# Francis-Fan-create/SCaSML_GP

Hardware: AMD Instinct MI355X
Metric: Euler-Maruyama path-steps/sec + L2 rel-error, Grad_Dependent_Nonlinear d=100 n=3 (higher is better)
Workload: dtype f32

## Files before the change

scasml_gp_amd/csrc/gp_eval_compat_mfma.hip:

```cpp
#include <stdlib.h>
#include <type_traits>

#include "gp_common.hpp"
#include "gp_mfma16.hpp"

namespace scasml {

constexpr int kHutch = 5;

typedef _Float16 h16x2 __attribute__((ext_vector_type(2)));
typedef float f32x2 __attribute__((ext_vector_type(2)));

struct CompatIdxF {
    int32_t i[kHutch];
};

struct GpCompatArgs {
    const float *points;
    const float *model;
    int32_t idx[kHutch];
    float4 *out4;
    float *lap;
    int64_t n_inf;
    int32_t n_pad, kp, d, first_bdy_tile;
    float a, sigma, mu;
    int32_t eq_id;
    int32_t round_out;
    const uint8_t *site_kinds;
    int64_t rows_per_site;
    const int32_t *site_order;
    int32_t n_listed;
    int32_t tail_packed;
};

template <bool R16>
struct Pair {
    using T = std::conditional_t<R16, h16x2, f32x2>;
    T v;
    __device__ __forceinline__ Pair(float a, float b) {
        if constexpr (R16) v = __builtin_convertvector((f32x2){a, b}, h16x2);
        else v = (f32x2){a, b};
    }
    __device__ __forceinline__ float lo() const { return (float)v.x; }
    __device__ __forceinline__ float hi() const { return (float)v.y; }
};

__device__ __forceinline__ float pin(float x) {
    asm("" : "+v"(x));
    return x;
}

static inline bool compat_tail_packed(int d, int kp) {
    const int r = d + 1 - (kp - 16);
    return 2 * (r > 0 ? r : 0) + 4 <= 16;
}

template <int KS, int PLANES, bool PACK>
__device__ __forceinline__ void compat_mfma_lam(const float4 *lds_a, const s16x8 (&xb)[PLANES][KS], f32x16 &acc, int lane, float acc0) {
#pragma unroll
    for (int r = 0; r < 16; ++r) acc[r] = acc0;
    constexpr int NA = PLANES == 2 ? 1 : 2;
    Frag a[NA];
    if constexpr (NA == 2) a[0].f = lds_a[lane];
#pragma unroll
    for (int s = 0; s < KS; ++s) {
        const int cur = NA == 2 ? (s & 1) : 0, nxt = cur ^ 1;
        if constexpr (NA == 2) {
            if (s + 1 < KS) a[nxt].f = lds_a[(s + 1) * 64 + lane];
        } else {
            a[0].f = lds_a[s * 64 + lane];
        }
        Frag b0;
        b0.v = xb[0][s];
        if constexpr (PLANES == 2) {
            if (!(PACK && s == KS - 1)) {
                Frag b1;
                b1.v = xb[1][s];
                acc = __builtin_amdgcn_mfma_f32_32x32x16_f16(a[cur].h, b1.h, acc, 0, 0, 0);
            }
        }
        acc = __builtin_amdgcn_mfma_f32_32x32x16_f16(a[cur].h, b0.h, acc, 0, 0, 0);
        __builtin_amdgcn_sched_barrier(0);
    }
}

struct CompatPoint {
    float sx, tx, ax0, sx2, wxa, wxb;
};
struct CompatConsts {
    float a, ad, c4, c10;
};

template <int GEOM, int FORM, bool BDY, bool R16>
__device__ __forceinline__ void compat_epilogue(const float *rows_lds, const f32x16 &lam, const f32x16 &G, int half, const CompatPoint &p,
                                                const CompatConsts &c, float &au, float &at, float &ad, float &al) {
    const float4 *cb = reinterpret_cast<const float4 *>(__builtin_assume_aligned(rows_lds + 4 * 8 * half, 16));
    constexpr int NQ = (BDY || GEOM == 1) ? 1 : 2;
    float4 q[1][NQ];
    auto fetch = [&](int r, float4 (&dst)[NQ]) {
        const int row = (r & 3) + 8 * (r >> 2);
#pragma unroll
        for (int i = 0; i < NQ; ++i) dst[i] = cb[row * 2 + i];
    };
#pragma unroll
    for (int r = 0; r < 16; ++r) {
        const int cur = 0;
        fetch(r, q[0]);
        __builtin_amdgcn_sched_barrier(0);
        const float kap = pin(__builtin_amdgcn_exp2f(lam[r]));
        if constexpr (GEOM == 0) {
            const float vsy = q[cur][0].x, vty = q[cur][0].y, c0 = q[cur][0].z;
            if constexpr (BDY && FORM == 1) {
                const Pair<R16> k0(kap, 0.0f);
                au = fmaf(c0, k0.lo(), au);
            } else {
                const float pp = p.tx - vty, ss = p.sx - vsy;
                const float e1 = pin(pp * kap), e2 = pin(ss * kap);
                if constexpr (BDY) {
                    const Pair<R16> k01(kap, e1), k2(e2, 0.0f);
                    au = fmaf(c0, k01.lo(), au);
                    if constexpr (FORM == 0) at = fmaf(-c0, k01.hi(), at);
                    if constexpr (FORM != 1) ad = fmaf(-c0, k2.lo(), ad);
                } else {
                    const float cL = q[cur][0].w, ct = q[cur][1].x, cS = q[cur][1].y;
                    if constexpr (FORM == 1) {
                        const Pair<R16> k01(kap, e1), k2(e2, 0.0f);
                        au = fmaf(cS, k2.lo(), fmaf(ct, k01.hi(), fmaf(c0, k01.lo(), au)));
                    } else {
                        const float e4 = pin(pp * e2);
                        const float e5 = pin(fmaf(-ss, e2, c.ad * kap));
                        if constexpr (FORM == 2) {
                            const Pair<R16> k01(kap, e1), k24(e2, e4), k5(e5, 0.0f);
                            au = fmaf(cS, k24.lo(), fmaf(ct, k01.hi(), fmaf(c0, k01.lo(), au)));
                            ad = fmaf(cS, k5.lo(), fmaf(-ct, k24.hi(), fmaf(-c0, k24.lo(), ad)));
                        } else {
                            const float e3 = fmaf(-pp, e1, c.a * kap);
                            const float g0 = G[r];
                            const float e6 = fmaf(g0, g0 - c.c4, -c.c10) * kap;
                            const Pair<R16> k01(kap, e1), k23(e2, e3), k45(e4, e5), k6(e6, 0.0f);
                            au = fmaf(cS, k23.lo(), fmaf(ct, k01.hi(), fmaf(c0, k01.lo(), au)));
                            at = fmaf(-cS, k45.lo(), fmaf(ct, k23.hi(), fmaf(-c0, k01.hi(), at)));
                            ad = fmaf(cS, k45.hi(), fmaf(-ct, k45.lo(), fmaf(-c0, k23.lo(), ad)));
                            al = fmaf(cL, k6.lo(), al);
                        }
                    }
                }
            }
        } else if constexpr (GEOM == 1) {
            const float vsy1 = q[cur][0].x, vay0 = q[cur][0].y, vwy1 = q[cur][0].z, cL = q[cur][0].w;
            const float g1 = G[r];
            const float f1 = pin(g1 * kap);
            if constexpr (FORM == 1) {
                const Pair<R16> k1(f1, 0.0f);
                au = fmaf(cL, k1.lo(), au);
            } else {
                const float m = fmaf(-(p.sx - vsy1), g1, p.wxb - vwy1);
                const float f3 = pin(m * kap);
                if constexpr (FORM == 2) {
                    const Pair<R16> k13(f1, f3);
                    au = fmaf(cL, k13.lo(), au);
                    ad = fmaf(cL, k13.hi(), ad);
                } else {
                    const float f2 = (p.tx - vay0) * f1;
                    const Pair<R16> k12(f1, f2), k3(f3, 0.0f);
                    au = fmaf(cL, k12.lo(), au);
                    at = fmaf(-cL, k12.hi(), at);
                    ad = fmaf(cL, k3.lo(), ad);
                }
            }
        } else {
            const float vsy = q[cur][0].x, vty = q[cur][0].y, vwy2 = q[cur][0].z, c0 = q[cur][0].w;
            const float g2 = G[r];
            const float h1 = g2 * kap;
            if constexpr (BDY) {
                const Pair<R16> k1(h1, 0.0f);
                al = fmaf(c0, k1.lo(), al);
            } else {
                const float ct = q[cur][1].x, cS = q[cur][1].y;
                const float h2 = (p.ax0 - vty) * h1;
                const float m = fmaf(-(p.sx2 - vsy), g2, p.wxa - vwy2);
                const float h3 = m * kap;
                const Pair<R16> k12(h1, h2), k3(h3, 0.0f);
                al = fmaf(-cS, k3.lo(), fmaf(ct, k12.hi(), fmaf(c0, k12.lo(), al)));
            }
        }
    }
}

template <int GEOM, int FORM, bool BDY>
__device__ __forceinline__ void compat_epilogue_fact(const float *rows_lds, const f32x16 &lam, const f32x16 &G, int half, const CompatPoint &p,
                                                     const CompatConsts &c, float &au, float &at, float &ad, float &al) {
    const float4 *cb = reinterpret_cast<const float4 *>(__builtin_assume_aligned(rows_lds + 4 * 8 * half, 16));
    constexpr int Q0 = GEOM == 2 ? 1 : 0;
    constexpr int NQ = (GEOM == 0 && !BDY) ? 2 : 1;
    float4 q[2][NQ];
    auto fetch = [&](int r, float4 (&dst)[NQ]) {
        const int row = (r & 3) + 8 * (r >> 2);
#pragma unroll
        for (int i = 0; i < NQ; ++i) dst[i] = cb[row * 2 + Q0 + i];
    };
    fetch(0, q[0]);
#pragma unroll
    for (int r = 0; r < 16; ++r) {
        const int cur = r & 1, nxt = cur ^ 1;
        if (r + 1 < 16) fetch(r + 1, q[nxt]);
        #ifndef SCASML_FACT_NOSCHED
        __builtin_amdgcn_sched_barrier(0);
#endif
        const float kap = __builtin_amdgcn_exp2f(lam[r]);
        if constexpr (GEOM == 0) {
            const float vsy = q[cur][0].x, vty = q[cur][0].y, c0 = q[cur][0].z;
            if constexpr (BDY) {
                const float F = c0 * kap;
                au += F;
                if constexpr (FORM == 0) at = fmaf(-(p.tx - vty), F, at);
                if constexpr (FORM != 1) ad = fmaf(-(p.sx - vsy), F, ad);
            } else {
                const float cL = q[cur][0].w, ct = q[cur][1].x, cS = q[cur][1].y;
                const float pp = p.tx - vty, ss = p.sx - vsy;
                const float E = fmaf(ct, pp, fmaf(cS, ss, c0));
                au = fmaf(kap, E, au);
                if constexpr (FORM != 1) ad = fmaf(kap, fmaf(-ss, E, q[cur][1].w), ad);
                if constexpr (FORM == 0) {
                    at = fmaf(kap, fmaf(-pp, E, q[cur][1].z), at);
                    const float g0 = G[r];
                    al = fmaf(cL * kap, fmaf(g0, g0 - c.c4, -c.c10), al);
                }
            }
        } else if constexpr (GEOM == 1) {
            const float vsy1 = q[cur][0].x, vay0 = q[cur][0].y, vwy1 = q[cur][0].z, cL = q[cur][0].w;
            const float v = cL * kap;
            if constexpr (FORM == 1) {
                au = fmaf(v, G[r], au);
            } else {
                const float w = v * G[r];
                au += w;
                ad = fmaf(-(p.sx - vsy1), w, fmaf(v, p.wxb - vwy1, ad));
                if constexpr (FORM == 0) at = fmaf(-(p.tx - vay0), w, at);
            }
        } else {
            const float ct = q[cur][0].x, cS = q[cur][0].y, e0 = q[cur][0].z, cSw = q[cur][0].w;
            if constexpr (BDY) {
                al = fmaf(kap * G[r], e0, al);
            } else {
                const float E2 = fmaf(ct, p.ax0, fmaf(cS, p.sx2, e0));
                const float t = fmaf(cS, p.wxa, -cSw);
                al = fmaf(kap, fmaf(G[r], E2, -t), al);
            }
        }
    }
}

constexpr int kStageTail = 256 + 256;

template <int KS, bool R16, int PLANES, bool PACK>
__device__ __forceinline__ void compat_mfma_sweep(const GpCompatArgs g) {
    static_assert(PLANES == 2 || !R16, "the as-coded form keeps both point planes");
#ifndef SCASML_COMPAT_NSLOT
#define SCASML_COMPAT_NSLOT 3
#endif
    constexpr int WPB = 4, NSLOT = SCASML_COMPAT_NSLOT, AHEAD = 2;
    constexpr int STAGE = KS * 256 + kStageTail;
    constexpr int NCHUNK = STAGE / 256;
    constexpr int CLO = NCHUNK / WPB, CREM = NCHUNK % WPB;
    extern __shared__ __attribute__((aligned(16))) float lds[];
    const int lane = threadIdx.x & 63, wv = threadIdx.x >> 6;
    const int col = lane & 31, half = lane >> 5;
    const int64_t blk = blockIdx.x;
    int64_t p0 = (blk * WPB + wv) * 32;
    const int n_tiles = g.n_pad / 32;
    const int nb0 = g.first_bdy_tile < n_tiles ? g.first_bdy_tile : n_tiles;

    int form_listed = -1;
    if (g.site_order) {
        const int64_t wps = g.rows_per_site >> 5;
        bool all_u = true, all_ud = true;
        for (int w = 0; w < WPB; ++w) {
            const int64_t vs = (blk * WPB + w) / wps;
            if (vs >= g.n_listed) continue;
            const int k = g.site_kinds ? g.site_kinds[g.site_order[vs]] : 0;
            if (!(k == 1 || k == 3)) all_u = false;
            if (!(k == 1 || k == 3 || k == 4)) all_ud = false;
        }
        form_listed = all_u ? 1 : (all_ud ? 2 : 0);
        const int64_t vw = blk * WPB + wv, vs = vw / wps;
        p0 = vs < g.n_listed ? (int64_t)g.site_order[vs] * g.rows_per_site + (vw - vs * wps) * 32 : g.n_inf;
    }

    p0 = ((int64_t)__builtin_amdgcn_readfirstlane((int32_t)(p0 >> 32)) << 32) | (uint32_t)__builtin_amdgcn_readfirstlane((int32_t)p0);

    if (!g.site_order && g.site_kinds && g.rows_per_site >= 32) {
        const int64_t b0 = blk * WPB * 32;
        if (b0 < g.n_inf) {
            const int64_t b1 = (b0 + WPB * 32 < g.n_inf ? b0 + WPB * 32 : g.n_inf) - 1;
            bool unowned = true;
            for (int64_t s = b0 / g.rows_per_site; s <= b1 / g.rows_per_site; ++s)
                if (g.site_kinds[s] != 2) unowned = false;
            if (unowned) return;
        }
    }
    int form = 0;
    if (g.site_order) {
        form = form_listed;
    } else if (g.site_kinds && g.rows_per_site >= 32) {
        const int64_t b0 = blk * WPB * 32;
        const int64_t b1 = (b0 + WPB * 32 < g.n_inf ? b0 + WPB * 32 : g.n_inf) - 1;
        if (b0 < g.n_inf) {
            bool all_u = true, all_ud = true;
            for (int64_t s = b0 / g.rows_per_site; s <= b1 / g.rows_per_site; ++s) {
                const int k = g.site_kinds[s];
                if (k == 2) continue;
                if (!(k == 1 || k == 3)) all_u = false;
                if (!(k == 1 || k == 3 || k == 4)) all_ud = false;
            }
            form = all_u ? 1 : (all_ud ? 2 : 0);
        }
    }
    form = __builtin_amdgcn_readfirstlane(form);
    const int GD = form == 0 ? 3 : 2, GB = form == 0 ? 2 : 1;
    const int n_stages = nb0 * GD + (n_tiles - nb0) * GB;

    const int wvs = __builtin_amdgcn_readfirstlane(wv);
    const bool extra = wvs < CREM;
    const uint32_t lds_base = __builtin_amdgcn_readfirstlane((uint32_t)(uintptr_t)lds);
    auto stage_src = [&](int s) -> const float * {
        int tile, geom;
        if (s < nb0 * GD) {
            tile = s / GD;
            geom = s - tile * GD;
        } else {
            const int t = s - nb0 * GD;
            tile = nb0 + t / GB;
            geom = form == 0 ? 2 * (t - (t / GB) * GB) : 0;
        }
        return g.model + ((int64_t)tile * 3 + geom) * STAGE;
    };
    auto stage = [&](int s) {
        const uint32_t dst = lds_base + (uint32_t)((s % NSLOT) * STAGE) * 4u;
        const float *src = stage_src(s);
        auto chunk = [&](int c) { glds16_asm(src + c * 256, (uint32_t)lane * 16u, dst + (uint32_t)c * 1024u); };
#pragma unroll
        for (int i = 0; i < CLO; ++i) chunk(wvs + i * WPB);
        if (CREM && extra) chunk(wvs + CLO * WPB);
    };
    auto rendezvous = [&](bool newest_may_fly) {
        if (newest_may_fly) {
            if (CREM && extra) {
                asm volatile("s_waitcnt vmcnt(%0)" ::"n"(CLO + 1) : "memory");
            } else {
                asm volatile("s_waitcnt vmcnt(%0)" ::"n"(CLO) : "memory");
            }
        } else {
            asm volatile("s_waitcnt vmcnt(0)" ::: "memory");
        }
        __builtin_amdgcn_s_barrier();
        asm volatile("" ::: "memory");
    };
    stage(0);
    if (n_stages > 1) stage(1);

    const float qs = 0.5f * 1.44269504088896341f / g.a, k1 = -qs;
    const float hh = (float)g.d / (float)kHutch;
    const float ha2 = hh * g.a * g.a;
    s16x8 xb[PLANES][KS];
    float acc0 = 0.0f;
    CompatPoint pt;
    Frag qa[1], qb[1];
    {
        int64_t row = p0 + col;
        if (row >= g.n_inf) row = g.n_inf - 1;
        const float *prow = g.points + row * g.kp;
        const float4 *src = reinterpret_cast<const float4 *>(prow + half * (8 * (KS - 1)));
        const float4 *src_tail = reinterpret_cast<const float4 *>(prow + 16 * (KS - 1) + (PACK ? 0 : 8 * half));
        float pn = 0.0f, ps = 0.0f;
        const float ptime = prow[g.d], px0 = prow[0];
        const float fold = 2.0f * g.a * g.a * qs;
        auto lo = [](float v) { return v - (float)(_Float16)v; };
        auto make_planes = [&](const float (&t)[8], Frag &fh, Frag &fl) {
#pragma unroll
            for (int c = 0; c < 4; ++c) {
                fh.u[c] = pack_h2(t[2 * c], t[2 * c + 1]);
                fl.u[c] = pack_h2(lo(t[2 * c]), lo(t[2 * c + 1]));
            }
        };
        float tlast[8];
#pragma unroll
        for (int s = 0; s < KS; ++s) {
            const bool last = s == KS - 1;
            const float4 q0 = last ? src_tail[0] : src[2 * s], q1 = last ? src_tail[1] : src[2 * s + 1];
            const float e[8] = {q0.x, q0.y, q0.z, q0.w, q1.x, q1.y, q1.z, q1.w};
            float t[8];
#pragma unroll
            for (int c2 = 0; c2 < 8; ++c2) {
                const float w = (PACK && last && half) ? 0.0f : e[c2];
                pn = fmaf(w, w, pn);
                ps += w;
                t[c2] = fold * e[c2];
            }
            if (last) {
#pragma unroll
                for (int c2 = 0; c2 < 8; ++c2) tlast[c2] = t[c2];
            } else {
                Frag fh, fl;
                make_planes(t, fh, fl);
                xb[0][s] = fh.v;
                if constexpr (PLANES == 2) xb[1][s] = fl.v;
            }
        }
        pn += __shfl_xor(pn, 32);
        ps += __shfl_xor(ps, 32);
        const float x2 = k1 * g.a * g.a * pn;
        if constexpr (PLANES == 1) {
            const bool packed = g.tail_packed != 0;
            tlast[5] = half ? (packed ? 0.0f : 1.0f) : tlast[5];
            tlast[6] = half ? (packed ? x2 : 1.0f) : (packed ? 1.0f : tlast[6]);
            tlast[7] = half ? (packed ? 0.0f : x2) : (packed ? 1.0f : tlast[7]);
            Frag fh, fl;
            make_planes(tlast, fh, fl);
            xb[0][KS - 1] = fh.v;
            acc0 = lo(x2);
        } else if constexpr (PACK) {
            Frag f;
#pragma unroll
            for (int c = 0; c < 3; ++c) {
                const uint32_t h2 = pack_h2(tlast[2 * c], tlast[2 * c + 1]);
                const uint32_t l2 = pack_h2(lo(tlast[2 * c]), lo(tlast[2 * c + 1]));
                f.u[c] = half ? l2 : h2;
            }
            f.u[3] = half ? pack_h2(x2, lo(x2)) : pack_h2(1.0f, 1.0f);
            xb[0][KS - 1] = f.v;
        } else {
            tlast[5] = half ? 1.0f : tlast[5];
            tlast[6] = half ? 1.0f : tlast[6];
            tlast[7] = half ? x2 : tlast[7];
            Frag fh, fl;
            make_planes(tlast, fh, fl);
            xb[0][KS - 1] = fh.v;
            xb[1][KS - 1] = fl.v;
        }
        pt.sx = g.a * (ps - ptime);
        pt.tx = g.a * ptime;
        pt.ax0 = g.a * px0;
        pt.sx2 = pt.sx - pt.ax0 + pt.tx;
        float ua[kHutch], ub[kHutch], sa = 0.0f, sb = 0.0f, na = 0.0f, nb = 0.0f;
#pragma unroll
        for (int j = 0; j < kHutch; ++j) {
            const float va = prow[g.idx[j] + 1], vb = prow[g.idx[j]];
            sa += va;
            sb += vb;
            na = fmaf(va, va, na);
            nb = fmaf(vb, vb, nb);
            ua[j] = -2.0f * ha2 * va;
            ub[j] = -2.0f * ha2 * vb;
        }
        pt.wxa = 2.0f * ha2 * sa;
        pt.wxb = 2.0f * ha2 * sb;
        auto qfrag = [&](const float (&u)[kHutch], float px, Frag &f) {
            auto hi = [](float v) { return (float)(_Float16)v; };
            if (half == 0) {
                f.u[0] = pack_h2(u[0], u[1]);
                f.u[1] = pack_h2(u[2], u[3]);
                f.u[2] = pack_h2(u[4], px);
                f.u[3] = pack_h2(px - hi(px), 1.0f);
            } else {
                f.u[0] = pack_h2(u[0] - hi(u[0]), u[1] - hi(u[1]));
                f.u[1] = pack_h2(u[2] - hi(u[2]), u[3] - hi(u[3]));
                f.u[2] = pack_h2(u[4] - hi(u[4]), 1.0f);
                f.u[3] = 0u;
            }
        };
        const float c5ah = (float)kHutch * g.a * hh;
        qfrag(ua, fmaf(ha2, na, -c5ah), qa[0]);
        qfrag(ub, fmaf(ha2, nb, -c5ah), qb[0]);
    }
    CompatConsts cc;
    cc.a = g.a;
    cc.ad = g.a * (float)g.d;
    cc.c4 = 4.0f * g.a * hh;
    cc.c10 = 10.0f * g.a * g.a * hh * hh;
    float au = 0.0f, at = 0.0f, ad = 0.0f, al = 0.0f;
    f32x16 acc, accG;
    uint32_t region;
    asm volatile("s_mov_b32 %0, -1" : "=s"(region));

    int s_now = 0;
    auto step = [&](auto geom_c, auto form_c, auto bdy_c) {
        constexpr int GEOM = decltype(geom_c)::value, FORM = decltype(form_c)::value;
        constexpr bool BDY = decltype(bdy_c)::value;
        constexpr bool NEEDG = GEOM != 0 || (FORM == 0 && !BDY);
        const int slot = s_now % NSLOT;
        if (s_now + AHEAD < n_stages) stage(s_now + AHEAD);
        const float *base = lds + slot * STAGE;
        if (region & 1) {
            compat_mfma_lam<KS, PLANES, PACK>(reinterpret_cast<const float4 *>(base), xb, acc, lane, acc0);
            if constexpr (NEEDG) {
                Frag aq;
                aq.f = reinterpret_cast<const float4 *>(base + KS * 256)[lane];
#pragma unroll
                for (int r = 0; r < 16; ++r) accG[r] = 0.0f;
                accG = __builtin_amdgcn_mfma_f32_32x32x16_f16(aq.h, GEOM == 1 ? qb[0].h : qa[0].h, accG, 0, 0, 0);
            }
        }
        if (region & 2) {
            if constexpr (R16) compat_epilogue<GEOM, FORM, BDY, true>(base + (KS + 1) * 256, acc, accG, half, pt, cc, au, at, ad, al);
            else compat_epilogue_fact<GEOM, FORM, BDY>(base + (KS + 1) * 256, acc, accG, half, pt, cc, au, at, ad, al);
        }
        rendezvous(s_now + AHEAD < n_stages);
        ++s_now;
    };
    using I0 = std::integral_constant<int, 0>;
    using I1 = std::integral_constant<int, 1>;
    using I2 = std::integral_constant<int, 2>;
    auto sweep = [&](auto form_c) {
        constexpr int FORM = decltype(form_c)::value;
        for (int jt = 0; jt < nb0; ++jt) {
            step(I0{}, form_c, std::false_type{});
            step(I1{}, form_c, std::false_type{});
            if constexpr (FORM == 0) step(I2{}, form_c, std::false_type{});
        }
        for (int jt = nb0; jt < n_tiles; ++jt) {
            step(I0{}, form_c, std::true_type{});
            if constexpr (FORM == 0) step(I2{}, form_c, std::true_type{});
        }
    };
    rendezvous(n_stages > 1);
    if (form == 2) sweep(I2{});
    else if (form == 1) sweep(I1{});
    else sweep(I0{});

    float u = au + __shfl_xor(au, 32);
    const float dt = at + __shfl_xor(at, 32);
    const float dv = ad + __shfl_xor(ad, 32);
    const float lp = al + __shfl_xor(al, 32);
    int col_out = col;
    if constexpr (R16) asm volatile("" : "+v"(col_out));
    const int64_t row = p0 + col_out;
    if (half == 0 && row < g.n_inf) {
        if (g.round_out) u = (float)(_Float16)u;
        float eps = dt + g.mu * dv + 0.5f * g.sigma * g.sigma * lp + eq_f<float>(g.eq_id, u, g.sigma * dv, g.sigma, (float)g.d);
        if (g.round_out) eps = (float)(_Float16)eps;
        g.out4[row] = make_float4(u, dv, eps, dt);
        if (g.lap) g.lap[row] = lp;
    }
}

template <int KS, int BPC, bool R16, int PLANES>
__global__ __launch_bounds__(256, BPC) void gp_eval_compat_mfma_kernel(const GpCompatArgs g) {
    compat_mfma_sweep<KS, R16, PLANES, false>(g);
}

template <int KS, int BPC, bool R16, int PLANES>
__global__ __launch_bounds__(256, BPC) void gp_eval_compat_mfma_tail_kernel(const GpCompatArgs g) {
    compat_mfma_sweep<KS, R16, PLANES, true>(g);
}

__global__ void gp_compat_pack_mfma_kernel(int d, float a, const float *x_dom, int n_dom, const float *x_bdy, int n_bdy, const double *rv,
                                           CompatIdxF ix, float *model, int n_pad, int kp, int packed) {
    const int j = blockIdx.x * blockDim.x + threadIdx.x;
    if (j >= n_pad) return;
    const int N = n_dom + n_bdy, D = d + 1, KS = kp / 16;
    const float *src = j < n_dom ? x_dom + (int64_t)j * D : (j < N ? x_bdy + (int64_t)(j - n_dom) * D : nullptr);
    auto y = [&](int k) { return src ? src[k] : 0.0f; };
    const float qs = 0.5f * 1.44269504088896341f / a, k1 = -qs;
    const float hh = (float)d / (float)kHutch, ha2 = hh * a * a;
    float ny = 0.0f, sy = 0.0f;
    for (int k = 0; k < D; ++k) ny = fmaf(y(k), y(k), ny);
    for (int k = 0; k < d; ++k) sy += y(k);
    const float ay = k1 * a * a * ny;
    const _Float16 ayh = (_Float16)ay;
    const float ayl = ay - (float)ayh;
    float c0 = 0.0f, cL = 0.0f, ct = 0.0f, cS = 0.0f;
    if (j < n_dom) {
        c0 = (float)rv[j];
        cL = (float)rv[N + j];
        ct = (float)rv[N + n_dom + j];
        cS = (float)rv[N + 2 * n_dom + j];
    } else if (j < N) {
        c0 = (float)rv[j];
    }
    const int tile = j / 32, i = j % 32;
    const int stage_floats = KS * 256 + kStageTail;
    for (int g = 0; g < 3; ++g) {
        float *blk = model + ((int64_t)tile * 3 + g) * stage_floats;
        uint16_t *planes = reinterpret_cast<uint16_t *>(blk);
        auto yg = [&](int k) { return g == 0 ? y(k) : (g == 1 ? y((k + 1) % D) : y((k + D - 1) % D)); };
        for (int s = 0; s < KS; ++s) {
            for (int c = 0; c < 16; ++c) {
                const int k = s < KS - 1 ? (c >> 3) * 8 * (KS - 1) + 8 * s + (c & 7)
                                         : 16 * s + (packed && c >= 8 ? c - 8 : c);
                float v = k <= d ? yg(k) : 0.0f;
                if (s == KS - 1) {
                    if (packed) v = (c & 7) < 6 ? v : (c == 6 ? (float)ayh : (c == 7 ? ayl : 1.0f));
                    else v = c < 13 ? v : (c == 13 ? (float)ayh : (c == 14 ? ayl : 1.0f));
                }
                planes[(((int64_t)s * 64 + (c >> 3) * 32 + i) * 8) + (c & 7)] = __builtin_bit_cast(unsigned short, (_Float16)v);
            }
        }
        float yq[kHutch], nq = 0.0f, sq = 0.0f;
        for (int q = 0; q < kHutch; ++q) {
            yq[q] = y(ix.i[q] + (g == 2 ? 0 : 1));
            nq = fmaf(yq[q], yq[q], nq);
            sq += yq[q];
        }
        const float py = ha2 * nq;
        const _Float16 pyh = (_Float16)py;
        uint16_t *qf = reinterpret_cast<uint16_t *>(blk + KS * 256);
        auto put = [&](int h, int e, float v) { qf[(h * 32 + i) * 8 + e] = __builtin_bit_cast(unsigned short, (_Float16)v); };
        for (int q = 0; q < kHutch; ++q) {
            put(0, q, yq[q]);
            put(1, q, yq[q]);
        }
        put(0, 5, 1.0f);
        put(0, 6, 1.0f);
        put(0, 7, (float)pyh);
        put(1, 5, py - (float)pyh);
        put(1, 6, 0.0f);
        put(1, 7, 0.0f);
        float *rc = blk + (KS + 1) * 256 + i * 8;
        for (int q = 0; q < 8; ++q) rc[q] = 0.0f;
        if (g == 0) {
            rc[0] = a * sy;
            rc[1] = a * y(d);
            rc[2] = c0;
            rc[3] = cL;
            rc[4] = ct;
            rc[5] = cS;
            rc[6] = a * ct;
            rc[7] = a * (float)d * cS;
        } else if (g == 1) {
            rc[0] = a * (sy - y(0) + y(d));
            rc[1] = a * y(0);
            rc[2] = 2.0f * ha2 * sq;
            rc[3] = cL;
        } else {
            rc[0] = a * sy;
            rc[1] = a * y(d);
            rc[2] = 2.0f * ha2 * sq;
            rc[3] = c0;
            rc[4] = ct;
            rc[5] = cS;
            rc[6] = fmaf(-cS, rc[0], fmaf(-ct, rc[1], c0));
            rc[7] = cS * rc[2];
        }
    }
}

template <int KS, bool R16, int PLANES, bool PACK>
static int launch_compat(const GpCompatArgs &g, hipStream_t s) {
    constexpr int REGS = 4 * PLANES * KS + (R16 ? 72 : 90);
    constexpr size_t lds_bytes = SCASML_COMPAT_NSLOT * (size_t)(KS * 256 + kStageTail) * sizeof(float);
    constexpr int BPC_REGS = REGS <= 128 ? 4 : (REGS <= 164 ? 3 : 2), BPC_LDS = (int)(160 * 1024 / lds_bytes);
    constexpr int BPC = BPC_REGS < BPC_LDS ? BPC_REGS : BPC_LDS;
    const int64_t waves = g.site_order ? (int64_t)g.n_listed * (g.rows_per_site >> 5) : (g.n_inf + 31) / 32;
    const int64_t blocks = (waves + 3) / 4;
    if (blocks == 0) return 0;
    if (blocks > 0x7FFFFFFF) return fail(SCASML_ERR_UNSUPPORTED, "gp_eval_compat_sites: too many points");
    static_assert(lds_bytes * BPC <= 160 * 1024, "LDS slots exceed 160 KiB");
    void (*kern)(const GpCompatArgs) = gp_eval_compat_mfma_kernel<KS, BPC, R16, PLANES>;
    if constexpr (PACK) kern = gp_eval_compat_mfma_tail_kernel<KS, BPC, R16, PLANES>;
    static_assert(PLANES == 2 || !PACK, "one plane: one kernel for both column maps");
    if (lds_bytes > 64 * 1024) {
        if (hipFuncSetAttribute(reinterpret_cast<const void *>(kern), hipFuncAttributeMaxDynamicSharedMemorySize, (int)lds_bytes) != hipSuccess)
            return fail(SCASML_ERR_HIP, "gp_eval_compat_sites: cannot reserve %zu bytes of LDS", lds_bytes);
    }
    hipLaunchKernelGGL(kern, dim3((unsigned)blocks), dim3(256), lds_bytes, s, g);
    return check_launch("gp_eval_compat_sites launch");
}

template <bool R16, int PLANES>
static int launch_compat_ks(const GpCompatArgs &g, hipStream_t s) {
    const bool packed = PLANES == 2 && g.tail_packed;
    switch (g.kp / 16) {
#define SCASML_CASE(K) \
    case K:                                                                                \
        if constexpr (PLANES == 2) {                                                       \
            if (packed) return launch_compat<K, R16, PLANES, true>(g, s);                   \
        }                                                                                  \
        return launch_compat<K, R16, PLANES, false>(g, s);
        SCASML_CASE(1) SCASML_CASE(2) SCASML_CASE(3) SCASML_CASE(4) SCASML_CASE(5) SCASML_CASE(6) SCASML_CASE(7) SCASML_CASE(8)
        SCASML_CASE(9) SCASML_CASE(10) SCASML_CASE(11) SCASML_CASE(12) SCASML_CASE(13) SCASML_CASE(14) SCASML_CASE(15) SCASML_CASE(16)
#undef SCASML_CASE
    }
    return fail(SCASML_ERR_UNSUPPORTED, "gp_eval_compat_sites: kp=%d", g.kp);
}

static int check_idx5(const int32_t *idx_h, int d, int32_t (&out)[kHutch], const char *who) {
    if (!idx_h) return fail(SCASML_ERR_ARG, "%s: idx is null", who);
    for (int j = 0; j < kHutch; ++j) {
        if (idx_h[j] < 0 || idx_h[j] >= d) return fail(SCASML_ERR_ARG, "%s: idx[%d] = %d outside [0, d)", who, j, idx_h[j]);
        for (int q = 0; q < j; ++q)
            if (idx_h[q] == idx_h[j]) return fail(SCASML_ERR_ARG, "%s: idx has a repeated entry %d", who, idx_h[j]);
        out[j] = idx_h[j];
    }
    return 0;
}

}

using namespace scasml;

extern "C" int64_t scasml_gp_compat_model_floats(int32_t d, int32_t n_pad) {
    const int64_t kp = scasml_point_stride(d);
    return (int64_t)(n_pad / SCASML_GP_TILE) * 3 * ((kp / 16) * 256 + kStageTail);
}

extern "C" int scasml_gp_compat_pack_mfma(int32_t d, float a, const float *x_dom, int32_t n_dom, const float *x_bdy, int32_t n_bdy,
                                          const double *rv, const int32_t *idx_h, float *model_out, void *stream) {
    if (!x_dom || !rv || !model_out || (n_bdy > 0 && !x_bdy)) return fail(SCASML_ERR_ARG, "gp_compat_pack_mfma: null argument");
    if (d < kHutch || d > SCASML_MAX_DIM || n_dom < 1 || n_bdy < 0) return fail(SCASML_ERR_ARG, "gp_compat_pack_mfma: bad sizes (d >= %d needed)", kHutch);
    CompatIdxF ix;
    if (int rc = check_idx5(idx_h, d, ix.i, "gp_compat_pack_mfma")) return rc;
    const int n_pad = (n_dom + n_bdy + 31) / 32 * 32;
    const int kp = scasml_point_stride(d);
    hipLaunchKernelGGL(gp_compat_pack_mfma_kernel, dim3((n_pad + 63) / 64), dim3(64), 0, (hipStream_t)stream, d, a, x_dom, n_dom, x_bdy, n_bdy,
                       rv, ix, model_out, n_pad, kp, compat_tail_packed(d, kp) ? 1 : 0);
    return check_launch("gp_compat_pack_mfma launch");
}

static int eval_compat_sites(int32_t d, float a, float sigma_eq, float mu_eq, int32_t eq_id, const float *model, int32_t n_dom,
                             int32_t n_bdy, const int32_t *idx_h, int32_t round16, float x_bound, const float *points, int64_t n_inf,
                             int64_t rows_per_site, const uint8_t *site_kinds, const int32_t *site_order, int32_t n_listed, float *out4, float *lap,
                             void *stream);

extern "C" int scasml_gp_eval_compat_sites(int32_t d, float a, float sigma_eq, float mu_eq, int32_t eq_id, const float *model, int32_t n_dom,
                                           int32_t n_bdy, const int32_t *idx_h, int32_t round16, float x_bound, const float *points, int64_t n_inf,
                                           int64_t rows_per_site, const uint8_t *site_kinds, float *out4, float *lap, void *stream) {
    return eval_compat_sites(d, a, sigma_eq, mu_eq, eq_id, model, n_dom, n_bdy, idx_h, round16, x_bound, points, n_inf, rows_per_site, site_kinds, nullptr,
                             0, out4, lap, stream);
}

extern "C" int scasml_gp_eval_compat_site_list(int32_t d, float a, float sigma_eq, float mu_eq, int32_t eq_id, const float *model, int32_t n_dom,
                                               int32_t n_bdy, const int32_t *idx_h, int32_t round16, float x_bound, const float *points, int64_t n_inf,
                                               int64_t rows_per_site, const uint8_t *site_kinds, const int32_t *site_order, int32_t n_listed,
                                               float *out4, float *lap, void *stream) {
    if (!site_order || n_listed < 0) return fail(SCASML_ERR_ARG, "gp_eval_compat_site_list: null or negative site list");
    if (rows_per_site < 32 || (rows_per_site & 31)) return fail(SCASML_ERR_ARG, "gp_eval_compat_site_list: rows_per_site must be a positive multiple of 32");
    if (n_inf % rows_per_site) return fail(SCASML_ERR_ARG, "gp_eval_compat_site_list: n_inf must be a whole number of sites");
    if (n_listed > n_inf / rows_per_site) return fail(SCASML_ERR_ARG, "gp_eval_compat_site_list: %d listed sites, the buffer holds %lld", n_listed, (long long)(n_inf / rows_per_site));
    if (n_listed == 0) return 0;
    return eval_compat_sites(d, a, sigma_eq, mu_eq, eq_id, model, n_dom, n_bdy, idx_h, round16, x_bound, points, n_inf, rows_per_site, site_kinds, site_order,
                             n_listed, out4, lap, stream);
}

static int eval_compat_sites(int32_t d, float a, float sigma_eq, float mu_eq, int32_t eq_id, const float *model, int32_t n_dom,
                             int32_t n_bdy, const int32_t *idx_h, int32_t round16, float x_bound, const float *points, int64_t n_inf,
                             int64_t rows_per_site, const uint8_t *site_kinds, const int32_t *site_order, int32_t n_listed, float *out4, float *lap,
                             void *stream) {
    if (n_inf == 0) return 0;
    if (!model || !points || !out4 || n_inf < 0) return fail(SCASML_ERR_ARG, "gp_eval_compat_sites: bad argument");
    if (d < kHutch || d > SCASML_MAX_DIM || n_dom < 1 || n_bdy < 0) return fail(SCASML_ERR_ARG, "gp_eval_compat_sites: bad sizes");
    if (site_kinds && rows_per_site < 1) return fail(SCASML_ERR_ARG, "gp_eval_compat_sites: rows_per_site must be positive");
    if (!eq_known(eq_id)) return fail(SCASML_ERR_UNSUPPORTED, "gp_eval_compat_sites: unknown equation id %d", eq_id);
    const float xb = x_bound > 0.0f ? x_bound : 2.0f;
    if (0.7213f * a * xb * xb * (float)(d + 1) > 3.0e4f)
        return fail(SCASML_ERR_UNSUPPORTED, "gp_eval_compat_sites: a = %g with |x_k| <= %g is outside the fp16 range at d = %d; use scasml_gp_eval_compat",
                    (double)a, (double)xb, d);
    GpCompatArgs g;
    if (int rc = check_idx5(idx_h, d, g.idx, "gp_eval_compat_sites")) return rc;
    g.points = points;
    g.model = model;
    g.out4 = reinterpret_cast<float4 *>(out4);
    g.lap = lap;
    g.n_inf = n_inf;
    g.n_pad = (n_dom + n_bdy + 31) / 32 * 32;
    g.kp = scasml_point_stride(d);
    g.d = d;
    g.first_bdy_tile = (n_dom + SCASML_GP_TILE - 1) / SCASML_GP_TILE;
    g.a = a;
    g.sigma = sigma_eq;
    g.mu = mu_eq;
    g.eq_id = eq_id;
    g.round_out = (round16 & 2) ? 1 : 0;
    g.site_kinds = site_kinds;
    g.rows_per_site = rows_per_site;
    g.site_order = site_order;
    g.n_listed = n_listed;
    g.tail_packed = compat_tail_packed(d, g.kp) ? 1 : 0;
    hipStream_t s = (hipStream_t)stream;
    if (round16 & 1) {
        if (round16 & 4) return fail(SCASML_ERR_ARG, "gp_eval_compat_sites: round16 bit 2 (one point plane) is the geometry mode's option, not the as-coded form's");
        return launch_compat_ks<true, 2>(g, s);
    }
    return (round16 & 4) ? launch_compat_ks<false, 1>(g, s) : launch_compat_ks<false, 2>(g, s);
}
```

Baseline: 481.0 million.

## Pair lone epilogue terms, park Q fragments in LDS, and trim register pressure

The epilogue now pairs consecutive rows' single-term products into one packed half pair instead of padding with zero, and prefetches the next row's LDS coefficients one row ahead for non-domain geometries. In the R16 path, the Q fragments are parked in a static LDS area and reloaded rather than held in registers. Several scalar constants are forced uniform, and lane and half indices are recomputed late to shorten live ranges. LDS moves from dynamic to static allocation capped at 64 KiB. The aim is to cut VGPR pressure and packed-conversion work, at the cost of extra LDS traffic and asm barriers that constrain scheduling.

```diff
diff --git a/scasml_gp_amd/csrc/gp_eval_compat_mfma.hip b/scasml_gp_amd/csrc/gp_eval_compat_mfma.hip
--- a/scasml_gp_amd/csrc/gp_eval_compat_mfma.hip
+++ b/scasml_gp_amd/csrc/gp_eval_compat_mfma.hip
@@ -96,52 +96,74 @@
                                                 const CompatConsts &c, float &au, float &at, float &ad, float &al) {
     const float4 *cb = reinterpret_cast<const float4 *>(__builtin_assume_aligned(rows_lds + 4 * 8 * half, 16));
     constexpr int NQ = (BDY || GEOM == 1) ? 1 : 2;
-    float4 q[1][NQ];
+#ifndef SCASML_COMPAT_ROW_AHEAD
+#define SCASML_COMPAT_ROW_AHEAD 1
+#endif
+    constexpr bool AHEAD = SCASML_COMPAT_ROW_AHEAD && GEOM != 0;
+    float4 q[AHEAD ? 2 : 1][NQ];
     auto fetch = [&](int r, float4 (&dst)[NQ]) {
         const int row = (r & 3) + 8 * (r >> 2);
 #pragma unroll
         for (int i = 0; i < NQ; ++i) dst[i] = cb[row * 2 + i];
     };
+    if constexpr (AHEAD) fetch(0, q[0]);
+    float held_v = 0.0f, held_c = 0.0f;
+    auto lone = [&](int r, float v, float coef, float &sum, auto &&rest) {
+        if (r & 1) {
+            const Pair<R16> k(held_v, v);
+            sum = fmaf(held_c, k.lo(), sum);
+            rest();
+            sum = fmaf(coef, k.hi(), sum);
+        } else {
+            rest();
+            held_v = v;
+            held_c = coef;
+        }
+    };
+    auto none = [] {};
 #pragma unroll
     for (int r = 0; r < 16; ++r) {
-        const int cur = 0;
-        fetch(r, q[0]);
-        __builtin_amdgcn_sched_barrier(0);
+        const int cur = AHEAD ? (r & 1) : 0;
+        if constexpr (AHEAD) {
+            if (r + 1 < 16) fetch(r + 1, q[cur ^ 1]);
+        } else {
+            fetch(r, q[0]);
+        }
+        if (!(r & 1)) __builtin_amdgcn_sched_barrier(0);
         const float kap = pin(__builtin_amdgcn_exp2f(lam[r]));
         if constexpr (GEOM == 0) {
             const float vsy = q[cur][0].x, vty = q[cur][0].y, c0 = q[cur][0].z;
             if constexpr (BDY && FORM == 1) {
-                const Pair<R16> k0(kap, 0.0f);
-                au = fmaf(c0, k0.lo(), au);
+                lone(r, kap, c0, au, none);
             } else {
                 const float pp = p.tx - vty, ss = p.sx - vsy;
                 const float e1 = pin(pp * kap), e2 = pin(ss * kap);
                 if constexpr (BDY) {
-                    const Pair<R16> k01(kap, e1), k2(e2, 0.0f);
+                    const Pair<R16> k01(kap, e1);
                     au = fmaf(c0, k01.lo(), au);
                     if constexpr (FORM == 0) at = fmaf(-c0, k01.hi(), at);
-                    if constexpr (FORM != 1) ad = fmaf(-c0, k2.lo(), ad);
+                    lone(r, e2, -c0, ad, none);
                 } else {
                     const float cL = q[cur][0].w, ct = q[cur][1].x, cS = q[cur][1].y;
                     if constexpr (FORM == 1) {
-                        const Pair<R16> k01(kap, e1), k2(e2, 0.0f);
-                        au = fmaf(cS, k2.lo(), fmaf(ct, k01.hi(), fmaf(c0, k01.lo(), au)));
+                        const Pair<R16> k01(kap, e1);
+                        lone(r, e2, cS, au, [&] { au = fmaf(ct, k01.hi(), fmaf(c0, k01.lo(), au)); });
                     } else {
                         const float e4 = pin(pp * e2);
                         const float e5 = pin(fmaf(-ss, e2, c.ad * kap));
                         if constexpr (FORM == 2) {
-                            const Pair<R16> k01(kap, e1), k24(e2, e4), k5(e5, 0.0f);
+                            const Pair<R16> k01(kap, e1), k24(e2, e4);
                             au = fmaf(cS, k24.lo(), fmaf(ct, k01.hi(), fmaf(c0, k01.lo(), au)));
-                            ad = fmaf(cS, k5.lo(), fmaf(-ct, k24.hi(), fmaf(-c0, k24.lo(), ad)));
+                            lone(r, e5, cS, ad, [&] { ad = fmaf(-ct, k24.hi(), fmaf(-c0, k24.lo(), ad)); });
                         } else {
                             const float e3 = fmaf(-pp, e1, c.a * kap);
                             const float g0 = G[r];
                             const float e6 = fmaf(g0, g0 - c.c4, -c.c10) * kap;
-                            const Pair<R16> k01(kap, e1), k23(e2, e3), k45(e4, e5), k6(e6, 0.0f);
+                            const Pair<R16> k01(kap, e1), k23(e2, e3), k45(e4, e5);
                             au = fmaf(cS, k23.lo(), fmaf(ct, k01.hi(), fmaf(c0, k01.lo(), au)));
                             at = fmaf(-cS, k45.lo(), fmaf(ct, k23.hi(), fmaf(-c0, k01.hi(), at)));
                             ad = fmaf(cS, k45.hi(), fmaf(-ct, k45.lo(), fmaf(-c0, k23.lo(), ad)));
-                            al = fmaf(cL, k6.lo(), al);
+                            lone(r, e6, cL, al, none);
                         }
                     }
                 }
@@ -151,8 +173,7 @@
             const float g1 = G[r];
             const float f1 = pin(g1 * kap);
             if constexpr (FORM == 1) {
-                const Pair<R16> k1(f1, 0.0f);
-                au = fmaf(cL, k1.lo(), au);
+                lone(r, f1, cL, au, none);
             } else {
                 const float m = fmaf(-(p.sx - vsy1), g1, p.wxb - vwy1);
                 const float f3 = pin(m * kap);
@@ -162,10 +183,10 @@
                     ad = fmaf(cL, k13.hi(), ad);
                 } else {
                     const float f2 = (p.tx - vay0) * f1;
-                    const Pair<R16> k12(f1, f2), k3(f3, 0.0f);
+                    const Pair<R16> k12(f1, f2);
                     au = fmaf(cL, k12.lo(), au);
                     at = fmaf(-cL, k12.hi(), at);
-                    ad = fmaf(cL, k3.lo(), ad);
+                    lone(r, f3, cL, ad, none);
                 }
             }
         } else {
@@ -173,15 +194,14 @@
             const float g2 = G[r];
             const float h1 = g2 * kap;
             if constexpr (BDY) {
-                const Pair<R16> k1(h1, 0.0f);
-                al = fmaf(c0, k1.lo(), al);
+                lone(r, h1, c0, al, none);
             } else {
                 const float ct = q[cur][1].x, cS = q[cur][1].y;
                 const float h2 = (p.ax0 - vty) * h1;
                 const float m = fmaf(-(p.sx2 - vsy), g2, p.wxa - vwy2);
                 const float h3 = m * kap;
-                const Pair<R16> k12(h1, h2), k3(h3, 0.0f);
-                al = fmaf(-cS, k3.lo(), fmaf(ct, k12.hi(), fmaf(c0, k12.lo(), al)));
+                const Pair<R16> k12(h1, h2);
+                lone(r, h3, -cS, al, [&] { al = fmaf(ct, k12.hi(), fmaf(c0, k12.lo(), al)); });
             }
         }
     }
@@ -253,19 +273,27 @@
 
 constexpr int kStageTail = 256 + 256;
 
+#ifndef SCASML_COMPAT_NSLOT
+#define SCASML_COMPAT_NSLOT 3
+#endif
+constexpr int kQParkWave = 2 * 64 * 4;
+template <int KS, bool R16>
+constexpr int compat_lds_floats() {
+    return SCASML_COMPAT_NSLOT * (KS * 256 + kStageTail) + (R16 ? 4 * kQParkWave : 0);
+}
+
 template <int KS, bool R16, int PLANES, bool PACK>
 __device__ __forceinline__ void compat_mfma_sweep(const GpCompatArgs g) {
     static_assert(PLANES == 2 || !R16, "the as-coded form keeps both point planes");
-#ifndef SCASML_COMPAT_NSLOT
-#define SCASML_COMPAT_NSLOT 3
-#endif
     constexpr int WPB = 4, NSLOT = SCASML_COMPAT_NSLOT, AHEAD = 2;
     constexpr int STAGE = KS * 256 + kStageTail;
     constexpr int NCHUNK = STAGE / 256;
     constexpr int CLO = NCHUNK / WPB, CREM = NCHUNK % WPB;
-    extern __shared__ __attribute__((aligned(16))) float lds[];
+    constexpr bool QLDS = R16;
+    __shared__ __attribute__((aligned(16))) float lds[compat_lds_floats<KS, R16>()];
     const int lane = threadIdx.x & 63, wv = threadIdx.x >> 6;
-    const int col = lane & 31, half = lane >> 5;
+    const int col = lane & 31;
+    const int half = (int)__builtin_amdgcn_mbcnt_lo(0x80000000u, 0u);
     const int64_t blk = blockIdx.x;
     int64_t p0 = (blk * WPB + wv) * 32;
     const int n_tiles = g.n_pad / 32;
@@ -321,8 +349,9 @@
     const int n_stages = nb0 * GD + (n_tiles - nb0) * GB;
 
     const int wvs = __builtin_amdgcn_readfirstlane(wv);
+    int lane_s = lane, half_s = half;
     const bool extra = wvs < CREM;
-    const uint32_t lds_base = __builtin_amdgcn_readfirstlane((uint32_t)(uintptr_t)lds);
+    const uint32_t lds_base = (uint32_t)(uintptr_t)lds;
     auto stage_src = [&](int s) -> const float * {
         int tile, geom;
         if (s < nb0 * GD) {
@@ -338,7 +367,7 @@
     auto stage = [&](int s) {
         const uint32_t dst = lds_base + (uint32_t)((s % NSLOT) * STAGE) * 4u;
         const float *src = stage_src(s);
-        auto chunk = [&](int c) { glds16_asm(src + c * 256, (uint32_t)lane * 16u, dst + (uint32_t)c * 1024u); };
+        auto chunk = [&](int c) { glds16_asm(src + c * 256, (uint32_t)lane_s * 16u, dst + (uint32_t)c * 1024u); };
 #pragma unroll
         for (int i = 0; i < CLO; ++i) chunk(wvs + i * WPB);
         if (CREM && extra) chunk(wvs + CLO * WPB);
@@ -366,6 +395,7 @@
     float acc0 = 0.0f;
     CompatPoint pt;
     Frag qa[1], qb[1];
+    float4 *qpark = reinterpret_cast<float4 *>(lds + NSLOT * STAGE) + wvs * (kQParkWave / 4);
     {
         int64_t row = p0 + col;
         if (row >= g.n_inf) row = g.n_inf - 1;
@@ -455,6 +485,7 @@
         }
         pt.wxa = 2.0f * ha2 * sa;
         pt.wxb = 2.0f * ha2 * sb;
+        if constexpr (PLANES == 1) asm volatile("" : "+v"(pt.ax0), "+v"(pt.sx2), "+v"(pt.wxa));
         auto qfrag = [&](const float (&u)[kHutch], float px, Frag &f) {
             auto hi = [](float v) { return (float)(_Float16)v; };
             if (half == 0) {
@@ -472,12 +503,22 @@
         const float c5ah = (float)kHutch * g.a * hh;
         qfrag(ua, fmaf(ha2, na, -c5ah), qa[0]);
         qfrag(ub, fmaf(ha2, nb, -c5ah), qb[0]);
-    }
+        if constexpr (QLDS) {
+            qpark[lane] = qa[0].f;
+            qpark[64 + lane] = qb[0].f;
+        }
+    }
+    auto late_lane = [](float after) {
+        int x;
+        asm volatile("v_mbcnt_lo_u32_b32 %0, -1, 0\n\tv_mbcnt_hi_u32_b32 %0, -1, %0" : "=v"(x) : "v"(after));
+        return x;
+    };
+    auto uni = [](float v) { return __builtin_bit_cast(float, __builtin_amdgcn_readfirstlane(__builtin_bit_cast(int, v))); };
     CompatConsts cc;
     cc.a = g.a;
-    cc.ad = g.a * (float)g.d;
-    cc.c4 = 4.0f * g.a * hh;
-    cc.c10 = 10.0f * g.a * g.a * hh * hh;
+    cc.ad = uni(g.a * (float)g.d);
+    cc.c4 = uni(4.0f * g.a * hh);
+    cc.c10 = uni(10.0f * g.a * g.a * hh * hh);
     float au = 0.0f, at = 0.0f, ad = 0.0f, al = 0.0f;
     f32x16 acc, accG;
     uint32_t region;
@@ -492,18 +533,20 @@
         if (s_now + AHEAD < n_stages) stage(s_now + AHEAD);
         const float *base = lds + slot * STAGE;
         if (region & 1) {
-            compat_mfma_lam<KS, PLANES, PACK>(reinterpret_cast<const float4 *>(base), xb, acc, lane, acc0);
+            compat_mfma_lam<KS, PLANES, PACK>(reinterpret_cast<const float4 *>(base), xb, acc, lane_s, acc0);
             if constexpr (NEEDG) {
                 Frag aq;
-                aq.f = reinterpret_cast<const float4 *>(base + KS * 256)[lane];
+                aq.f = reinterpret_cast<const float4 *>(base + KS * 256)[lane_s];
 #pragma unroll
                 for (int r = 0; r < 16; ++r) accG[r] = 0.0f;
-                accG = __builtin_amdgcn_mfma_f32_32x32x16_f16(aq.h, GEOM == 1 ? qb[0].h : qa[0].h, accG, 0, 0, 0);
+                Frag bq = GEOM == 1 ? qb[0] : qa[0];
+                if constexpr (QLDS) bq.f = qpark[(GEOM == 1 ? 64 : 0) + lane];
+                accG = __builtin_amdgcn_mfma_f32_32x32x16_f16(aq.h, bq.h, accG, 0, 0, 0);
             }
         }
         if (region & 2) {
-            if constexpr (R16) compat_epilogue<GEOM, FORM, BDY, true>(base + (KS + 1) * 256, acc, accG, half, pt, cc, au, at, ad, al);
-            else compat_epilogue_fact<GEOM, FORM, BDY>(base + (KS + 1) * 256, acc, accG, half, pt, cc, au, at, ad, al);
+            if constexpr (R16) compat_epilogue<GEOM, FORM, BDY, true>(base + (KS + 1) * 256, acc, accG, half_s, pt, cc, au, at, ad, al);
+            else compat_epilogue_fact<GEOM, FORM, BDY>(base + (KS + 1) * 256, acc, accG, half_s, pt, cc, au, at, ad, al);
         }
         rendezvous(s_now + AHEAD < n_stages);
         ++s_now;
@@ -513,6 +556,10 @@
     using I2 = std::integral_constant<int, 2>;
     auto sweep = [&](auto form_c) {
         constexpr int FORM = decltype(form_c)::value;
+        if constexpr (PLANES == 1) {
+            lane_s = late_lane(au);
+            half_s = lane_s >> 5;
+        }
         for (int jt = 0; jt < nb0; ++jt) {
             step(I0{}, form_c, std::false_type{});
             step(I1{}, form_c, std::false_type{});
@@ -528,16 +575,34 @@
     else if (form == 1) sweep(I1{});
     else sweep(I0{});
 
-    float u = au + __shfl_xor(au, 32);
-    const float dt = at + __shfl_xor(at, 32);
-    const float dv = ad + __shfl_xor(ad, 32);
-    const float lp = al + __shfl_xor(al, 32);
+    auto other_half = [&](float v) {
+        if constexpr (PLANES == 1) {
+            const int peer = (late_lane(v) ^ 32) << 2;
+            return __builtin_bit_cast(float, __builtin_amdgcn_ds_bpermute(peer, __builtin_bit_cast(int, v)));
+        } else {
+            return __shfl_xor(v, 32);
+        }
+    };
+    float u = au + other_half(au);
+    const float dt = at + other_half(at);
+    const float dv = ad + other_half(ad);
+    const float lp = al + other_half(al);
     int col_out = col;
     if constexpr (R16) asm volatile("" : "+v"(col_out));
+    int half_out = half;
+    float fd = (float)g.d;
+    if constexpr (PLANES == 1) {
+        const int l = late_lane(u);
+        col_out = l & 31;
+        half_out = l >> 5;
+        int d_late = g.d;
+        asm volatile("" : "+s"(d_late));
+        fd = (float)d_late;
+    }
     const int64_t row = p0 + col_out;
-    if (half == 0 && row < g.n_inf) {
+    if (half_out == 0 && row < g.n_inf) {
         if (g.round_out) u = (float)(_Float16)u;
-        float eps = dt + g.mu * dv + 0.5f * g.sigma * g.sigma * lp + eq_f<float>(g.eq_id, u, g.sigma * dv, g.sigma, (float)g.d);
+        float eps = dt + g.mu * dv + 0.5f * g.sigma * g.sigma * lp + eq_f<float>(g.eq_id, u, g.sigma * dv, g.sigma, fd);
         if (g.round_out) eps = (float)(_Float16)eps;
         g.out4[row] = make_float4(u, dv, eps, dt);
         if (g.lap) g.lap[row] = lp;
@@ -648,22 +713,18 @@
 template <int KS, bool R16, int PLANES, bool PACK>
 static int launch_compat(const GpCompatArgs &g, hipStream_t s) {
     constexpr int REGS = 4 * PLANES * KS + (R16 ? 72 : 90);
-    constexpr size_t lds_bytes = SCASML_COMPAT_NSLOT * (size_t)(KS * 256 + kStageTail) * sizeof(float);
+    constexpr size_t lds_bytes = compat_lds_floats<KS, R16>() * sizeof(float);
     constexpr int BPC_REGS = REGS <= 128 ? 4 : (REGS <= 164 ? 3 : 2), BPC_LDS = (int)(160 * 1024 / lds_bytes);
     constexpr int BPC = BPC_REGS < BPC_LDS ? BPC_REGS : BPC_LDS;
     const int64_t waves = g.site_order ? (int64_t)g.n_listed * (g.rows_per_site >> 5) : (g.n_inf + 31) / 32;
     const int64_t blocks = (waves + 3) / 4;
     if (blocks == 0) return 0;
     if (blocks > 0x7FFFFFFF) return fail(SCASML_ERR_UNSUPPORTED, "gp_eval_compat_sites: too many points");
-    static_assert(lds_bytes * BPC <= 160 * 1024, "LDS slots exceed 160 KiB");
+    static_assert(lds_bytes * BPC <= 160 * 1024 && lds_bytes <= 64 * 1024, "LDS slots exceed 160 KiB per CU or 64 KiB per workgroup");
     void (*kern)(const GpCompatArgs) = gp_eval_compat_mfma_kernel<KS, BPC, R16, PLANES>;
     if constexpr (PACK) kern = gp_eval_compat_mfma_tail_kernel<KS, BPC, R16, PLANES>;
     static_assert(PLANES == 2 || !PACK, "one plane: one kernel for both column maps");
-    if (lds_bytes > 64 * 1024) {
-        if (hipFuncSetAttribute(reinterpret_cast<const void *>(kern), hipFuncAttributeMaxDynamicSharedMemorySize, (int)lds_bytes) != hipSuccess)
-            return fail(SCASML_ERR_HIP, "gp_eval_compat_sites: cannot reserve %zu bytes of LDS", lds_bytes);
-    }
-    hipLaunchKernelGGL(kern, dim3((unsigned)blocks), dim3(256), lds_bytes, s, g);
+    hipLaunchKernelGGL(kern, dim3((unsigned)blocks), dim3(256), 0, s, g);
     return check_launch("gp_eval_compat_sites launch");
 }
 
```

Measured after the change: 486.6 million (median of 6 runs). 1.2% higher.
